# tsinghua-fib-lab/DRL-urban-planning

Measured on NVIDIA H100. Metric: ppo_update_graph_samples_per_sec, higher is better.
Workload: dtype f32

## Files before the change

drl_urban_planning_b200/csrc/mlp_kernel.cuh:

```cuda
#pragma once
#include "sgnn_kernel.cuh"

namespace upb {

constexpr int M_NUM_W0 = 0;
constexpr int M_NUM_B0 = 3328;
constexpr int M_NUM_W1 = 3392;
constexpr int M_NUM_B1 = 4416;
constexpr int M_ENC_W = 4432;
constexpr int M_ENC_B = 4800;
constexpr int M_LU_W0 = 4816;
constexpr int M_LU_B0 = 6864;
constexpr int M_LU_W1 = 6896;
constexpr int M_RD_W0 = 6928;
constexpr int M_RD_B0 = 7440;
constexpr int M_RD_W1 = 7472;
constexpr int M_SVD = 51;
constexpr int M_VAL_W0 = 7504;
constexpr int M_VAL_B0 = 9136;
constexpr int M_VAL_W1 = 9168;
constexpr int M_VAL_B1 = 10192;
constexpr int M_VAL_W2 = 10224;
constexpr int M_VAL_B2 = 10256;
constexpr int M_NUM_PARAMS = 10257;
// ... 364 lines not shown
    float s0 = 0.f, s1 = 0.f;
    int i = 0;
    for (; i + 1 < n; i += 2) {
      s0 = fmaf(GH[(size_t)i * 16 + c], X[(size_t)i * FS + f], s0);
      s1 = fmaf(GH[(size_t)(i + 1) * 16 + c], X[(size_t)(i + 1) * FS + f], s1);
    }
    if (i < n) s0 = fmaf(GH[(size_t)i * 16 + c], X[(size_t)i * FS + f], s0);
    gacc(gp, M_ENC_W + idx, (s0 + s1) + sV[MV_GHC + c] * sV[MV_XCUR + f]);
  }
  if (tid < 16) gacc(gp, M_ENC_B + tid, sV[MV_T16 + tid] + sV[MV_GHC + tid]);
  __syncthreads();
}

constexpr int M_NSLICE = MlpRow::nslice;
static_assert(M_NSLICE == 81 && MG_ROW - (M_NSLICE - 1) * SLICE == 64,
              "tests/test_gpu_mlp_step.py runs the rl-mlp fused tail at grids of 80 / 81 / 82 CTAs around M_NSLICE: move them");
static_assert(M_NSLICE * SLICE <= G_ROW && M_NSLICE <= FLAG_STRIDE, "the SGNN exchange buffer holds the rl-mlp row");
static_assert(MT == 2 * SLICE, "two threads per column of a slice");

__device__ void mlp_fused_tail(const StepArgs& a, float* smem, unsigned stage_bits) {
  const int tid = threadIdx.x;
  const int nparts = gridDim.x;
  const int world = a.world, me = a.rank;
  const bool sys = world > 1;
  const unsigned par = a.seq & 1u;
  __shared__ TailShared sh;
  float* const mine = a.peers[me];
  const float* const pull = mine + (size_t)par * MAX_PEERS * G_ROW;
  const unsigned* const myflags = reinterpret_cast<const unsigned*>(mine + XCHG_FLAGS) + (size_t)par * MAX_PEERS * FLAG_STRIDE;
  tail_prologue(a, sh, stage_bits);
  const int c = tid & (SLICE - 1), half = tid >> 7;
  const int col0 = blockIdx.x * SLICE + c;
  float pm = 0.f, pv = 0.f, pp = 0.f;
  if (half == 0 && col0 < M_NUM_PARAMS) { pm = a.adam_m[col0]; pv = a.adam_v[col0]; pp = a.params_rw[col0]; }
  const unsigned flagword = tail_barrier(a);

  float* sHalf = smem;
  const int nq = nparts & ~3;
  for (int sl = blockIdx.x; sl < M_NSLICE; sl += gridDim.x) {
    const int col = sl * SLICE + c;
    const bool in_row = col < MG_ROW;
    const float* src = a.gpart + col + (size_t)(2 * half) * MG_ROW;
    float sa = 0.f, sb = 0.f;
    if (in_row) {
      int r = 0;
      for (; r + 16 <= nq; r += 16) {
        float t[8];
#pragma unroll
        for (int j = 0; j < 4; ++j) {
          t[2 * j] = __ldcg(src + (size_t)(r + 4 * j) * MG_ROW);
          t[2 * j + 1] = __ldcg(src + (size_t)(r + 4 * j + 1) * MG_ROW);
        }
#pragma unroll
        for (int j = 0; j < 4; ++j) { sa += t[2 * j]; sb += t[2 * j + 1]; }
      }
      for (; r < nq; r += 4) {
        const float x0 = __ldcg(src + (size_t)r * MG_ROW), x1 = __ldcg(src + (size_t)(r + 1) * MG_ROW);
        sa += x0; sb += x1;
      }
      if (half == 0)
        for (r = nq; r < nparts; ++r) sa += __ldcg(src + (size_t)r * MG_ROW);
    }
    const float pair = sa + sb;
    __syncthreads();
    if (half) sHalf[c] = pair;
    __syncthreads();
    if (half == 0 && in_row) {
      const float v = pair + sHalf[c];
      for (int r = 0; r < world; ++r) st_relaxed(sh.push[r] + col, v, sys);
    }
  }
  tail_release<MlpRow>(a, flagword, MT, sys);
  if (a.kl_stop) tail_kl_gate<MlpRow>(a, sh, pull, myflags, sys);

  tail_reduce_adam<MlpRow>(a, sh, pull, myflags, sys, c, half == 0, col0, pm, pv, pp);
  if (blockIdx.x == 0 && tid < 4) tail_write_steps(a, sh);
  tail_count_timeout(a, sh);
}

template <bool TRAIN>
__global__ void __launch_bounds__(MT, 1) k_mlp(const __grid_constant__ StepArgs a) {
  extern __shared__ __align__(16) float smem[];
  __shared__ __align__(8) uint64_t s_mbar[1];
  if constexpr (TRAIN) {
    if (a.kl_stop && kl_stop_set(a.kl_stop)) {
      skip_step<MlpRow>(a);
      return;
    }
  }
  if (threadIdx.x == 0) { mbar_init(s_mbar, 1); fence_mbar_init(); }
  for (int i = threadIdx.x; i < 10272; i += MT) smem[MS_P + i] = i < M_NUM_PARAMS ? a.params[i] : 0.f;
  for (int i = threadIdx.x; i < 384; i += MT) {
    const int f = i >> 4, c = i & 15;
    smem[MS_WET + i] = f < F ? a.params[M_ENC_W + c * F + f] : 0.f;
  }
  float* gp = nullptr;
  if constexpr (TRAIN) {
    gp = a.gpart + (size_t)blockIdx.x * MG_ROW;
    for (int i = threadIdx.x; i < MG_ROW; i += MT) gp[i] = 0.f;
  }
  __syncthreads();
  const BlobHeader& hd = *reinterpret_cast<const BlobHeader*>(a.blob);
  const GraphDesc* descs = reinterpret_cast<const GraphDesc*>(a.blob + hd.off_desc);
  float* scr = a.scratch + (size_t)blockIdx.x * a.scratch_stride;
  unsigned nstaged = 0;
  unsigned stage_bits = 0;
  for (int item = blockIdx.x; item < a.count; item += gridDim.x) {
    const int gid = a.ids ? a.ids[item] : item;
    const GraphDesc d = descs[gid];
    if (d.n > a.n_cap || d.e > a.e_cap || d.n < 1) {
      if (threadIdx.x == 0) {
        if constexpr (TRAIN) gp[MG_STATS + 7] += 1.f;
        if (a.out_value) a.out_value[gid] = CUDART_NAN_F;
        if (a.out_logp) a.out_logp[gid] = CUDART_NAN_F;
        if (a.out_entropy) a.out_entropy[gid] = CUDART_NAN_F;
      }
      if constexpr (!TRAIN) write_skipped_logit_row<MT>(a, gid, d.stage);
      continue;
    }
    stage_bits |= d.stage == 0 ? 1u : (d.stage == 1 ? 2u : 0u);
    const bool big = d.n > M_NS || 2 * d.e > M_AS || d.k > M_KS;
    mlp_graph<TRAIN>(a, hd, d, gid, smem, gp, scr, s_mbar, nstaged & 1u, big);
    if (!big) ++nstaged;
    __syncthreads();
  }
  if constexpr (TRAIN) {
    if (a.fuse_tail) mlp_fused_tail(a, smem, stage_bits);
  }
}

__global__ void __launch_bounds__(256) k_mlp_reduce(const float* __restrict__ gpart, int nparts, float* __restrict__ grad,
                                                    const unsigned int* kl_stop) {
  const int idx = blockIdx.x * 256 + threadIdx.x;
  if (kl_stop && kl_stop_set(kl_stop)) {
    if (idx < UPB_MLP_GRAD_STRIDE) write_skip_elem(grad, UPB_MLP_STAT_OFFSET, idx);
    return;
  }
  if (idx >= MG_ROW) return;
  write_grad_col<MlpRow>(grad, idx, column_sum4<MlpRow>(gpart, nparts, idx));
}

}
```

drl_urban_planning_b200/csrc/sgnn_kernel.cuh:

```cuda
#pragma once
#include <cuda_runtime.h>
#include <math_constants.h>
#include <stdint.h>

#include "blob.h"
#include "layout.h"
#include "optim_kernels.cuh"

namespace upb {

constexpr int NT = 512;
constexpr int NW = NT / 32;
constexpr int NS = 464;
constexpr int AS = 5632;
constexpr int KS = 160;
constexpr int CH = 96;
constexpr float MASK_FILL = -4294967296.0f;
constexpr float EPS_DEG = 1e-6f;

constexpr int S_WET = 0;
constexpr int S_BE = S_WET + 384;
constexpr int S_WPQ0 = S_BE + 16;
constexpr int S_B0 = S_WPQ0 + 512;
constexpr int S_WPQ1 = S_B0 + 16;
// ... 128 lines not shown
  const float* fixed_lp;
  const float* exps;
  float inv_batch, inv_ind;
  float clip_lo, clip_hi;
  float c_value, c_entropy;
  int diagnostics;
  float* out_value;
  float* out_logp;
  float* out_entropy;
  int* out_greedy;
  const float* uniforms;
  int* out_sample;
  float* gpart;
  float* scratch;
  size_t scratch_stride;
  int n_cap, e_cap;
  int fuse_tail;
  float* params_rw;
  float* grad_out;
  float* adam_m;
  float* adam_v;
  const long long* steps_in;
  long long* steps_out;
  unsigned int* gridbar;
  unsigned int bar_target;
  float lr, beta1, beta2, adam_eps;
  float weight_decay;
  int world, rank;
  unsigned int seq;
  float* const* peers;
  long long* stamps;
  const int* logit_rows;
  float* lu_logits;
  float* rd_logits;
  unsigned int* kl_stop;
  float kl_limit;
};

__device__ __forceinline__ float ex2_approx(float x) {
  float y;
  asm("ex2.approx.ftz.f32 %0, %1;" : "=f"(y) : "f"(x));
  return y;
}
__device__ __forceinline__ float rcp_approx(float x) {
  float y;
  asm("rcp.approx.ftz.f32 %0, %1;" : "=f"(y) : "f"(x));
  return y;
}
__device__ __forceinline__ float exp2a(float a) {
  const float t = fminf(fmaxf(a * 2.8853900817779268f, -115.41560327111707f), 115.41560327111707f);
  return ex2_approx(t);
}
__device__ __forceinline__ void cp_async16(void* smem_dst, const void* gsrc) {
  const unsigned d = (unsigned)__cvta_generic_to_shared(smem_dst);
  asm volatile("cp.async.cg.shared.global [%0], [%1], 16;" ::"r"(d), "l"(gsrc) : "memory");
}
__device__ __forceinline__ void cp_async_commit() { asm volatile("cp.async.commit_group;" ::: "memory"); }
__device__ __forceinline__ void cp_async_wait_all() { asm volatile("cp.async.wait_group 0;" ::: "memory"); }

__device__ __forceinline__ unsigned smem_u32(const void* p) { return (unsigned)__cvta_generic_to_shared(p); }
__device__ __forceinline__ void mbar_init(uint64_t* bar, unsigned count) {
  asm volatile("mbarrier.init.shared::cta.b64 [%0], %1;" ::"r"(smem_u32(bar)), "r"(count) : "memory");
}
__device__ __forceinline__ void fence_mbar_init() { asm volatile("fence.mbarrier_init.release.cluster;" ::: "memory"); }
__device__ __forceinline__ void fence_proxy_async() { asm volatile("fence.proxy.async;" ::: "memory"); }
__device__ __forceinline__ void mbar_expect_tx(uint64_t* bar, unsigned bytes) {
  asm volatile("mbarrier.arrive.expect_tx.shared::cta.b64 _, [%0], %1;" ::"r"(smem_u32(bar)), "r"(bytes) : "memory");
}
__device__ __forceinline__ void bulk_g2s(void* smem_dst, const void* gsrc, unsigned bytes, uint64_t* bar) {
  asm volatile("cp.async.bulk.shared::cluster.global.mbarrier::complete_tx::bytes [%0], [%1], %2, [%3];"
               ::"r"(smem_u32(smem_dst)), "l"(gsrc), "r"(bytes), "r"(smem_u32(bar)) : "memory");
}
__device__ __forceinline__ void mbar_wait(uint64_t* bar, unsigned parity) {
  asm volatile(
      "{\n\t.reg .pred p;\n\t"
      "WAIT_%=:\n\t"
      "mbarrier.try_wait.parity.shared::cta.b64 p, [%0], %1;\n\t"
      "@p bra DONE_%=;\n\t"
      "bra WAIT_%=;\n\t"
      "DONE_%=:\n\t}"
      ::"r"(smem_u32(bar)), "r"(parity) : "memory");
}

__device__ __forceinline__ float4 ld4(const float* p) { return *reinterpret_cast<const float4*>(p); }
__device__ __forceinline__ void st4(float* p, float4 v) { *reinterpret_cast<float4*>(p) = v; }
__device__ __forceinline__ float4 f4(float a) { return make_float4(a, a, a, a); }
__device__ __forceinline__ float4 operator+(float4 a, float4 b) { return make_float4(a.x + b.x, a.y + b.y, a.z + b.z, a.w + b.w); }
__device__ __forceinline__ float4 operator*(float4 a, float s) { return make_float4(a.x * s, a.y * s, a.z * s, a.w * s); }
__device__ __forceinline__ float4 operator*(float4 a, float4 b) { return make_float4(a.x * b.x, a.y * b.y, a.z * b.z, a.w * b.w); }
__device__ __forceinline__ float dot4(float4 a, float4 b) { return a.x * b.x + a.y * b.y + a.z * b.z + a.w * b.w; }
__device__ __forceinline__ float comp(const float4& v, int j) { return j == 0 ? v.x : j == 1 ? v.y : j == 2 ? v.z : v.w; }

struct F2x2 { float2 a, b; };
__device__ __forceinline__ float2 ffma2(float2 a, float2 b, float2 c) {
  return make_float2(__fmaf_rn(a.x, b.x, c.x), __fmaf_rn(a.y, b.y, c.y));
}
__device__ __forceinline__ float2 fmul2(float2 a, float2 b) { return make_float2(__fmul_rn(a.x, b.x), __fmul_rn(a.y, b.y)); }
__device__ __forceinline__ float2 fadd2(float2 a, float2 b) { return make_float2(__fadd_rn(a.x, b.x), __fadd_rn(a.y, b.y)); }
__device__ __forceinline__ F2x2 ldp(const float* p) {
  const float4 v = ld4(p);
  F2x2 r; r.a = make_float2(v.x, v.y); r.b = make_float2(v.z, v.w);
  return r;
}
template <bool SM>
struct RowBase {
  const float* p;
  unsigned a;
  __device__ __forceinline__ explicit RowBase(const float* base) : p(base), a(SM ? smem_u32(base) : 0u) {}
  __device__ __forceinline__ F2x2 row(unsigned k, int shift) const {
    if constexpr (SM) {
      float4 v;
      asm volatile("ld.shared.v4.f32 {%0, %1, %2, %3}, [%4];" : "=f"(v.x), "=f"(v.y), "=f"(v.z), "=f"(v.w) : "r"(a + (k << shift)));
      F2x2 r; r.a = make_float2(v.x, v.y); r.b = make_float2(v.z, v.w);
      return r;
    } else {
      return ldp(reinterpret_cast<const float*>(reinterpret_cast<const char*>(p) + ((size_t)k << shift)));
    }
  }
};
__device__ __forceinline__ float2 rcp2(float2 v) { return make_float2(rcp_approx(v.x), rcp_approx(v.y)); }
__device__ __forceinline__ float2 neg2(float2 v) { return make_float2(-v.x, -v.y); }

template <int TIER>
__device__ __forceinline__ float2 edge_den(float2 p, float2 q) {
  if constexpr (TIER == 2) {
    const float2 x = fadd2(p, q);
    return make_float2(__fadd_rn(exp2a(x.x), 1.f), __fadd_rn(exp2a(x.y), 1.f));
  } else {
    return ffma2(p, q, make_float2(1.f, 1.f));
  }
}
template <int TIER>
__device__ __forceinline__ void fwd_term(float2 epi, float2 eqi, float2 epk, float2 eqk, float2& s) {
  const float2 a = edge_den<TIER>(epi, eqk), b = edge_den<TIER>(epk, eqi);
  if (TIER > 0) s = fadd2(s, fadd2(rcp2(a), rcp2(b)));
  else s = ffma2(fadd2(a, b), rcp2(fmul2(a, b)), s);
}
template <int TIER>
__device__ __forceinline__ void bwd_term(float2 epi, float2 eqi, float2 epk, float2 eqk, float2 ge2, float2& aP,
                                         float2& aQ) {
  const float2 one = make_float2(1.f, 1.f);
  const float2 a = edge_den<TIER>(epi, eqk), b = edge_den<TIER>(epk, eqi);
  float2 r1, r2;
  if (TIER > 0) { r1 = rcp2(a); r2 = rcp2(b); }
  else { const float2 R = rcp2(fmul2(a, b)); r1 = fmul2(b, R); r2 = fmul2(a, R); }
  aP = ffma2(ge2, fmul2(r1, fadd2(one, neg2(r1))), aP);
  aQ = ffma2(ge2, fmul2(r2, fadd2(one, neg2(r2))), aQ);
}

__device__ __forceinline__ float warp_sum(float v) {
#pragma unroll
  for (int o = 16; o > 0; o >>= 1) v += __shfl_xor_sync(0xffffffffu, v, o);
  return v;
}
__device__ __forceinline__ float warp_max(float v) {
#pragma unroll
  for (int o = 16; o > 0; o >>= 1) v = fmaxf(v, __shfl_xor_sync(0xffffffffu, v, o));
  return v;
}

__device__ __forceinline__ float block_sum1(float v, float* red) {
  v = warp_sum(v);
  if ((threadIdx.x & 31) == 0) red[threadIdx.x >> 5] = v;
  __syncthreads();
  float s = 0.f;
#pragma unroll
// ... 1499 lines not shown
constexpr unsigned PEER_SPIN_LIMIT = 1u << 24;

__device__ __forceinline__ float ld_relaxed(const float* p, bool sys) {
  float v;
  if (sys) asm volatile("ld.relaxed.sys.global.f32 %0, [%1];" : "=f"(v) : "l"(p));
  else asm volatile("ld.relaxed.gpu.global.f32 %0, [%1];" : "=f"(v) : "l"(p));
  return v;
}
__device__ __forceinline__ void st_relaxed(float* p, float v, bool sys) {
  if (sys) asm volatile("st.relaxed.sys.global.f32 [%0], %1;" ::"l"(p), "f"(v) : "memory");
  else asm volatile("st.relaxed.gpu.global.f32 [%0], %1;" ::"l"(p), "f"(v) : "memory");
}
__device__ __forceinline__ unsigned ld_acquire(const unsigned* p, bool sys) {
  unsigned v;
  if (sys) asm volatile("ld.acquire.sys.global.u32 %0, [%1];" : "=r"(v) : "l"(p) : "memory");
  else asm volatile("ld.acquire.gpu.global.u32 %0, [%1];" : "=r"(v) : "l"(p) : "memory");
  return v;
}
__device__ __forceinline__ void st_release(unsigned* p, unsigned v, bool sys) {
  if (sys) asm volatile("st.release.sys.global.u32 [%0], %1;" ::"l"(p), "r"(v) : "memory");
  else asm volatile("st.release.gpu.global.u32 [%0], %1;" ::"l"(p), "r"(v) : "memory");
}

__device__ __forceinline__ void grid_arrive(unsigned int* ctr) {
  __syncthreads();
  if (threadIdx.x == 0) {
    __threadfence();
    atomicAdd(ctr, 1u);
  }
}
__device__ __forceinline__ void grid_wait(unsigned int* ctr, unsigned int target) {
  if (threadIdx.x == 0) {
    unsigned int v;
    do {
      asm volatile("ld.acquire.gpu.global.u32 %0, [%1];" : "=r"(v) : "l"(ctr) : "memory");
    } while ((int)(v - target) < 0);
    __threadfence();
  }
  __syncthreads();
}

__device__ __forceinline__ void adam_elem(const StepArgs& a, int i, float g, float m, float v, float p, float step_size,
                                          float bc2_sqrt) {
  const float w1 = 1.f - a.beta1, w2 = 1.f - a.beta2;
  if (a.weight_decay != 0.f) g = __fmaf_rn(a.weight_decay, p, g);
  m = __fadd_rn(m, __fmul_rn(w1, __fsub_rn(g, m)));
  v = __fadd_rn(__fmul_rn(v, a.beta2), __fmul_rn(__fmul_rn(w2, g), g));
  const float denom = __fadd_rn(__fdiv_rn(__fsqrt_rn(v), bc2_sqrt), a.adam_eps);
  a.params_rw[i] = __fadd_rn(p, __fmul_rn(-step_size, __fdiv_rn(m, denom)));
  a.adam_m[i] = m;
  a.adam_v[i] = v;
}

struct TailShared {
  float adam[12];
  long long steps[6];
  unsigned bits;
  int timeout;
  int stop;
  float* push[MAX_PEERS];
};

__device__ __forceinline__ void tail_prologue(const StepArgs& a, TailShared& sh, unsigned stage_bits) {
  const int tid = threadIdx.x;
  const unsigned par = a.seq & 1u;
  if (tid < a.world) sh.push[tid] = a.peers[tid] + ((size_t)par * MAX_PEERS + a.rank) * G_ROW;
  if (tid == 32) { sh.timeout = 0; sh.bits = 0u; sh.stop = 0; }
  if (tid == 0 && stage_bits) atomicOr(a.gridbar + 2 + par, stage_bits);
  if (tid == 1 && blockIdx.x == 0) a.gridbar[2 + (par ^ 1u)] = 0u;
  if (tid < 6) {
    const int seg = tid >> 1, live = tid & 1;
    const long long stp = a.steps_in[1 + seg] + live;
    const double bc1 = 1.0 - ipow((double)a.beta1, stp > 0 ? stp : 1);
    const double bc2 = 1.0 - ipow((double)a.beta2, stp > 0 ? stp : 1);
    sh.adam[tid * 2 + 0] = (float)((double)a.lr / bc1);
    sh.adam[tid * 2 + 1] = (float)sqrt(bc2);
    sh.steps[tid] = stp;
  }
}

__device__ __forceinline__ unsigned tail_barrier(const StepArgs& a) {
  grid_arrive(a.gridbar);
  grid_wait(a.gridbar, a.bar_target);
  unsigned mybits;
  asm volatile("ld.acquire.gpu.global.u32 %0, [%1];" : "=r"(mybits) : "l"(a.gridbar + 2 + (a.seq & 1u)) : "memory");
  return (a.seq << 2) | (mybits & 3u);
}

template <class L>
__device__ __forceinline__ void tail_release(const StepArgs& a, unsigned flagword, int nthreads, bool sys) {
  __syncthreads();
  const unsigned par = a.seq & 1u;
  const int nown = (L::nslice - (int)blockIdx.x + (int)gridDim.x - 1) / (int)gridDim.x;
  for (int idx = threadIdx.x; idx < a.world * nown; idx += nthreads) {
    const int r = idx % a.world, sl = blockIdx.x + (idx / a.world) * gridDim.x;
    unsigned* f = reinterpret_cast<unsigned*>(a.peers[r] + XCHG_FLAGS) + ((size_t)par * MAX_PEERS + a.rank) * FLAG_STRIDE + sl;
    if (sys) __threadfence_system(); else __threadfence();
    st_release(f, flagword, sys);
  }
}

__device__ __forceinline__ void tail_poll(const StepArgs& a, TailShared& sh, const unsigned* myflags, int r, int sl,
                                          bool sys) {
  unsigned polls = 0, f;
  while ((int)(((f = ld_acquire(myflags + (size_t)r * FLAG_STRIDE + sl, sys)) >> 2) - a.seq) < 0) {
    if (++polls >= PEER_SPIN_LIMIT) { sh.timeout = 1; break; }
  }
  if (f & 3u) atomicOr(&sh.bits, f & 3u);
}

template <class L>
__device__ __forceinline__ void tail_reduce_adam(const StepArgs& a, TailShared& sh, const float* pull,
                                                 const unsigned* myflags, bool sys, int c, bool active, int col0,
                                                 float pm, float pv, float pp) {
  const int world = a.world;
  for (int sl = blockIdx.x; sl < L::nslice; sl += gridDim.x) {
    if ((int)threadIdx.x < world) tail_poll(a, sh, myflags, threadIdx.x, sl, sys);
    __syncthreads();
    const bool live_lu = sh.bits & 1u, live_rd = sh.bits & 2u;
    const bool dead = sh.timeout != 0 || sh.stop;
    const int col = sl * SLICE + c;
    if (active && (L::row % SLICE == 0 || col < L::row)) {
      float v[MAX_PEERS];
#pragma unroll
      for (int p = 0; p < MAX_PEERS; ++p) v[p] = p < world ? ld_relaxed(pull + (size_t)p * G_ROW + col, sys) : 0.f;
      float s = v[0];
#pragma unroll
      for (int p = 1; p < MAX_PEERS; ++p) if (p < world) s += v[p];
      if (write_grad_col<L>(a.grad_out, col, s)) {
        int seg = 0;
        bool live = true;
        if (col >= L::lu_begin && col < L::rd_begin) { seg = 1; live = live_lu; }
        else if (col >= L::rd_begin && col < L::policy_end) { seg = 2; live = live_rd; }
        if (live && !dead) {
          if (col != col0) { pm = a.adam_m[col]; pv = a.adam_v[col]; pp = a.params_rw[col]; }
          adam_elem(a, col, s, pm, pv, pp, sh.adam[(seg * 2 + 1) * 2], sh.adam[(seg * 2 + 1) * 2 + 1]);
        }
      } else if (sh.stop && col == L::stats + KL_STOP_SLOT) {
        a.grad_out[L::stat_offset + KL_STOP_SLOT] = 1.f;
        *a.kl_stop = 1u;
      }
    }
    __syncthreads();
  }
}

__device__ __forceinline__ void tail_write_steps(const StepArgs& a, const TailShared& sh) {
  const int tid = threadIdx.x;
  const bool live_lu = sh.bits & 1u, live_rd = sh.bits & 2u;
  if (sh.timeout == 0 && !sh.stop)
    a.steps_out[tid] = tid == 0 ? a.steps_in[0] + 1
                                : sh.steps[(tid - 1) * 2 + (tid == 1 ? 1 : (tid == 2 ? (live_lu ? 1 : 0) : (live_rd ? 1 : 0)))];
  else
    a.steps_out[tid] = a.steps_in[tid];
}

__device__ __forceinline__ void tail_count_timeout(const StepArgs& a, const TailShared& sh) {
  if (threadIdx.x == 0 && sh.timeout) atomicAdd(a.gridbar + 6, 1u);
}

template <class L>
__device__ __noinline__ void tail_kl_gate(const StepArgs& a, TailShared& sh, const float* pull, const unsigned* myflags,
                                          bool sys) {
  if ((int)threadIdx.x < a.world) tail_poll(a, sh, myflags, threadIdx.x, L::stats / SLICE, sys);
  __syncthreads();
  if (threadIdx.x == 0) {
// ... 66 lines not shown
    }
  }
  const unsigned flagword = tail_barrier(a);
  UPB_TSTAMP(41);

  float* sPart = smem + 4096;
  for (int sl = blockIdx.x; sl < NSLICE; sl += gridDim.x) {
    const int lane = tid & 31, warp = tid >> 5, cg = warp & 3, rg = warp >> 2;
    const float* src = a.gpart + sl * SLICE + cg * 32 + lane;
    float s = 0.f;
    for (int r0 = rg; r0 < nparts; r0 += 160) {
      float t[40];
#pragma unroll
      for (int j = 0; j < 40; ++j) t[j] = r0 + 4 * j < nparts ? __ldcg(src + (size_t)(r0 + 4 * j) * G_ROW) : 0.f;
#pragma unroll
      for (int w = 1; w < 40; w <<= 1)
#pragma unroll
        for (int j = 0; j + w < 40; j += 2 * w) t[j] += t[j + w];
      s += t[0];
    }
    __syncthreads();
    sPart[rg * SLICE + cg * 32 + lane] = s;
    __syncthreads();
    if (tid < SLICE) {
      const float v = (sPart[tid] + sPart[SLICE + tid]) + (sPart[2 * SLICE + tid] + sPart[3 * SLICE + tid]);
      const int col = sl * SLICE + tid;
      for (int r = 0; r < world; ++r) st_relaxed(sh.push[r] + col, v, sys);
    }
  }
  tail_release<SgnnRow>(a, flagword, NT, sys);
  if (a.kl_stop) tail_kl_gate<SgnnRow>(a, sh, pull, myflags, sys);
  UPB_TSTAMP(42);

  tail_reduce_adam<SgnnRow>(a, sh, pull, myflags, sys, tid >> 2, part == 0, col0, pm, pv, pp);
  UPB_TSTAMP(43);
  if (!chain_cta) {
    tail_count_timeout(a, sh);
    return;
  }

  {
    constexpr int NCH = CHAIN_S1 - CHAIN_S0 + 1;
    if (tid < world * NCH) tail_poll(a, sh, myflags, tid % world, CHAIN_S0 + tid / world, sys);
    __syncthreads();
  }
  const bool dead = sh.timeout != 0 || sh.stop;
  if (tid < 4) tail_write_steps(a, sh);
  {
    float v0[MAX_PEERS], v1[MAX_PEERS];
#pragma unroll
    for (int p = 0; p < MAX_PEERS; ++p) {
      v0[p] = 0.f; v1[p] = 0.f;
      if (p < world) {
        v0[p] = ld_relaxed(pull + (size_t)p * G_ROW + G_QC + tid, sys);
        if (tid + NT < 816) v1[p] = ld_relaxed(pull + (size_t)p * G_ROW + G_QC + tid + NT, sys);
      }
    }
    float s0 = v0[0], s1 = v1[0];
#pragma unroll
    for (int p = 1; p < MAX_PEERS; ++p) if (p < world) { s0 += v0[p]; s1 += v1[p]; }
    sG[tid] = s0;
    if (tid + NT < 816) sG[tid + NT] = s1;
  }
  __syncthreads();
  if (tid < 256) attention_chain(tid, sG, sWin, sW3, sB, sOut, 256, sOut + 768, sOut + 1536, 16, sOut + 1584);
  __syncthreads();
#pragma unroll
  for (int j = 0; j < 4; ++j) {
    const int i = tid + j * NT;
    if (i < 1632) {
      const float g = sOut[i];
      a.grad_out[cdst[j]] = g;
      if (!dead) adam_elem(a, cdst[j], g, cm[j], cv[j], cp[j], sh.adam[2], sh.adam[3]);
    }
  }
  tail_count_timeout(a, sh);
  UPB_TSTAMP(44);
}

template <bool TRAIN>
__global__ void __launch_bounds__(NT, 1) k_sgnn(const __grid_constant__ StepArgs a) {
  extern __shared__ __align__(16) float smem[];
  __shared__ __align__(8) uint64_t s_mbar[4];
  if constexpr (TRAIN) {
    if (a.kl_stop && kl_stop_set(a.kl_stop)) {
      skip_step<SgnnRow>(a);
      return;
    }
  }
  const long long t_cta0 = a.stamps ? clock64() : 0;
  if (a.stamps && threadIdx.x == 0 && blockIdx.x == 0) {
    unsigned long long gt;
    asm volatile("mov.u64 %0, %%globaltimer;" : "=l"(gt));
    a.stamps[30] = t_cta0; a.stamps[32] = (long long)gt;
  }
  if (threadIdx.x == 0) {
    mbar_init(s_mbar + 0, 1); mbar_init(s_mbar + 1, 1); mbar_init(s_mbar + 2, 1); mbar_init(s_mbar + 3, 1);
    fence_mbar_init();
  }
  unsigned nstaged = 0;
  load_weights(a.params, smem);
  float* gp = nullptr;
  if constexpr (TRAIN) {
    gp = a.gpart + (size_t)blockIdx.x * G_ROW;
    for (int i = threadIdx.x; i < G_ROW / 4; i += NT) reinterpret_cast<float4*>(gp)[i] = f4(0.f);
  }
  __syncthreads();
  if (a.stamps && threadIdx.x == 0 && blockIdx.x < 160) a.stamps[64 + 160 + blockIdx.x] = clock64() - t_cta0;
  const BlobHeader& hd = *reinterpret_cast<const BlobHeader*>(a.blob);
  const GraphDesc* descs = reinterpret_cast<const GraphDesc*>(a.blob + hd.off_desc);
  float* scr = a.scratch + (size_t)blockIdx.x * a.scratch_stride;
  unsigned stage_bits = 0;
  for (int item = blockIdx.x; item < a.count; item += gridDim.x) {
    const int gid = a.ids ? a.ids[item] : item;
    const GraphDesc d = descs[gid];
    stage_bits |= 1u << (d.stage & 1);
    if (d.n > a.n_cap || d.e > a.e_cap || d.n < 1) {
      if (threadIdx.x == 0) {
        if constexpr (TRAIN) gacc(gp, G_STATS + 7, 1.f);
        if (a.out_value) a.out_value[gid] = CUDART_NAN_F;
        if (a.out_logp) a.out_logp[gid] = CUDART_NAN_F;
        if (a.out_entropy) a.out_entropy[gid] = CUDART_NAN_F;
      }
      if constexpr (!TRAIN) write_skipped_logit_row<NT>(a, gid, d.stage);
      continue;
    }
    if (item + (int)gridDim.x < a.count) prefetch_next_graph<TRAIN>(a, item + gridDim.x);
    const bool big = d.n > NS || 2 * d.e > AS || d.k > KS || d.ord_rounds > ORD_ROUNDS;
    if (big) graph_body<TRAIN, true>(a, hd, d, gid, smem, gp, scr, item == (int)(blockIdx.x + gridDim.x), s_mbar, 0u);
    else { graph_body<TRAIN, false>(a, hd, d, gid, smem, gp, scr, item == (int)(blockIdx.x + gridDim.x), s_mbar, nstaged & 1u); ++nstaged; }
    __syncthreads();
  }
  if (a.stamps && threadIdx.x == 0 && blockIdx.x < 160) a.stamps[64 + blockIdx.x] = clock64() - t_cta0;
  if (a.stamps && threadIdx.x == 0 && blockIdx.x == 0) {
    unsigned long long gt;
    asm volatile("mov.u64 %0, %%globaltimer;" : "=l"(gt));
    a.stamps[31] = clock64(); a.stamps[33] = (long long)gt;
  }
  if constexpr (TRAIN) {
    if (a.fuse_tail) fused_tail(a, smem, stage_bits);
  }
}

}
```

drl_urban_planning_b200/csrc/upb200.cu:

```cuda
#include <cuda_runtime.h>

#include <cmath>
#include <cstdio>
#include <cstring>
#include <new>
#include <string>
#include <utility>
#include <vector>

#include "../../include/upb200.h"
#include "blob.h"
#include "errors.h"
#include "layout.h"
#include "optim_kernels.cuh"
#include "sgnn_kernel.cuh"
#include "mlp_kernel.cuh"

using namespace upb;

struct Model {
  void (*train)(StepArgs);
  void (*infer)(StepArgs);
  int threads;
  size_t smem;
  int row;
  int num_params, encoder_end, policy_end, lu_begin, rd_begin, stat_offset, grad_stride;
  size_t (*scratch_floats)(int n_cap, int e_cap);
  void (*reduce)(const upb_ctx* ctx, int nparts, const float* params, float* grad, const unsigned int* kl_stop,
                 cudaStream_t s);
  bool peer_exchange;

  float* gpart = nullptr;
  float* scratch = nullptr;
  size_t scratch_stride = 0;
  float* adam_m = nullptr;
  float* adam_v = nullptr;
  long long* steps = nullptr;
  unsigned int* kl_stop = nullptr;
  int steps_cur = 0;
  bool clip_armed = true;
};

namespace {
void reduce_sgnn(const upb_ctx* ctx, int nparts, const float* params, float* grad, const unsigned int* kl_stop,
                 cudaStream_t s);
void reduce_mlp(const upb_ctx* ctx, int nparts, const float* params, float* grad, const unsigned int* kl_stop,
                cudaStream_t s);
}

struct upb_ctx {
  upb_config cfg;
  int num_sms = 0;
  int grid = 0;
  Model sgnn{k_sgnn<true>, k_sgnn<false>, NT, SMEM_BYTES, G_ROW, NUM_PARAMS, ENCODER_END, POLICY_END, P_LU_W0,
             P_RD_W0, UPB_STAT_OFFSET, UPB_GRAD_STRIDE, scratch_floats, reduce_sgnn, true};
  Model mlp{k_mlp<true>, k_mlp<false>, MT, M_SMEM_BYTES, MG_ROW, M_NUM_PARAMS, M_ENCODER_END, M_POLICY_END, M_LU_W0,
            M_RD_W0, UPB_MLP_STAT_OFFSET, UPB_MLP_GRAD_STRIDE, mlp_scratch_floats, reduce_mlp, false};
  float* gsum = nullptr;
  unsigned int* ticket = nullptr;
  unsigned int* gridbar = nullptr;
  unsigned int bar_total = 0;
  float weight_decay = 0.f;
  bool diagnostics = false;
  float kl_limit = 0.f;
  float clip_lo = 0.f, clip_hi = 0.f;
  int coop = 0;
  float* host_pinned = nullptr;
  int64_t launches = 0;
  bool profiling = false;
  long long* stamps = nullptr;
  std::vector<std::pair<cudaEvent_t, cudaEvent_t>> prof_events;
  size_t prof_used = 0;
  float* xchg = nullptr;
  int world = 1, rank = 0;
  unsigned int peer_seq = 0;
  std::vector<void*> peer_ptrs;
  float** peers_dev = nullptr;
};

namespace {

#define UPB_CUDA(call)                                                                       \
  do {                                                                                       \
    cudaError_t err__ = (call);                                                              \
    if (err__ != cudaSuccess) {                                                              \
      char buf__[512];                                                                       \
      snprintf(buf__, sizeof(buf__), "%s failed: %s (%s:%d)", #call, cudaGetErrorString(err__), \
               __FILE__, __LINE__);                                                          \
      return set_error(UPB_ERR_CUDA, buf__);                                                 \
    }                                                                                        \
  } while (0)

struct Slot {
  const char* name;
  int offset, rows, cols;
};
const Slot kSlots[] = {
    {"num_w0", P_NUM_W0, 64, 52},      {"num_b0", P_NUM_B0, 64, 0},     {"num_w1", P_NUM_W1, 16, 64},
    {"num_b1", P_NUM_B1, 16, 0},       {"enc_w", P_ENC_W, 16, 23},      {"enc_b", P_ENC_B, 16, 0},
    {"gcn0_w", P_GCN0_W, 16, 32},      {"gcn0_b", P_GCN0_B, 16, 0},     {"gcn1_w", P_GCN1_W, 16, 32},
    {"gcn1_b", P_GCN1_B, 16, 0},       {"mha_in_w", P_MHA_IN_W, 48, 16}, {"mha_in_b", P_MHA_IN_B, 48, 0},
    {"mha_out_w", P_MHA_OUT_W, 16, 16}, {"mha_out_b", P_MHA_OUT_B, 16, 0}, {"att_q_w", P_ATT_Q_W, 16, 16},
    {"att_q_b", P_ATT_Q_B, 16, 0},     {"att_k_w", P_ATT_K_W, 16, 16},  {"att_k_b", P_ATT_K_B, 16, 0},
    {"att_v_w", P_ATT_V_W, 16, 16},    {"att_v_b", P_ATT_V_B, 16, 0},   {"lu_w0", P_LU_W0, 32, 64},
    {"lu_b0", P_LU_B0, 32, 0},         {"lu_w1", P_LU_W1, 1, 32},       {"road_w0", P_RD_W0, 32, 16},
    {"road_b0", P_RD_B0, 32, 0},       {"road_w1", P_RD_W1, 1, 32},     {"val_w0", P_VAL_W0, 32, 67},
    {"val_b0", P_VAL_B0, 32, 0},       {"val_w1", P_VAL_W1, 32, 32},    {"val_b1", P_VAL_B1, 32, 0},
    {"val_w2", P_VAL_W2, 1, 32},       {"val_b2", P_VAL_B2, 1, 0},
};
constexpr int kNumSlots = sizeof(kSlots) / sizeof(kSlots[0]);

using ModelOf = Model upb_ctx::*;

int check_ctx(const upb_ctx* ctx, const char* who) {
  if (!ctx) return set_error(UPB_ERR_ARG, std::string(who) + ": null context");
  return UPB_OK;
}
int bad_argument(const char* who) { return set_error(UPB_ERR_ARG, std::string(who) + ": bad argument"); }

bool prof_begin(upb_ctx* ctx, cudaStream_t s) {
  if (!ctx->profiling) return false;
  if (ctx->prof_used == ctx->prof_events.size()) {
    cudaEvent_t a, b;
    if (cudaEventCreate(&a) != cudaSuccess || cudaEventCreate(&b) != cudaSuccess) return false;
    ctx->prof_events.emplace_back(a, b);
  }
  cudaEventRecord(ctx->prof_events[ctx->prof_used].first, s);
  return true;
}
void prof_end(upb_ctx* ctx, cudaStream_t s, bool on) {
  if (!on) return;
  cudaEventRecord(ctx->prof_events[ctx->prof_used].second, s);
  ctx->prof_used += 1;
}

bool clip_now(const upb_ctx* ctx, const Model& m) {
  return ctx->cfg.clip_mode == UPB_CLIP_ALWAYS || (ctx->cfg.clip_mode == UPB_CLIP_REFERENCE && m.clip_armed);
}

int model_init(upb_ctx* ctx, Model& m) {
  if (m.gpart) return UPB_OK;
  m.scratch_stride = (m.scratch_floats(ctx->cfg.n_cap, ctx->cfg.e_cap) + 63) & ~size_t(63);
  UPB_CUDA(cudaMalloc(&m.gpart, sizeof(float) * (size_t)ctx->grid * m.row));
  UPB_CUDA(cudaMalloc(&m.scratch, sizeof(float) * (size_t)ctx->grid * m.scratch_stride));
  UPB_CUDA(cudaMalloc(&m.adam_m, sizeof(float) * m.num_params));
  UPB_CUDA(cudaMalloc(&m.adam_v, sizeof(float) * m.num_params));
  UPB_CUDA(cudaMalloc(&m.steps, sizeof(long long) * 8));
  UPB_CUDA(cudaMalloc(&m.kl_stop, sizeof(unsigned int)));
  UPB_CUDA(cudaMemset(m.kl_stop, 0, sizeof(unsigned int)));
  UPB_CUDA(cudaMemset(m.adam_m, 0, sizeof(float) * m.num_params));
  UPB_CUDA(cudaMemset(m.adam_v, 0, sizeof(float) * m.num_params));
  UPB_CUDA(cudaMemset(m.steps, 0, sizeof(long long) * 8));
  UPB_CUDA(cudaMemset(m.scratch, 0, sizeof(float) * (size_t)ctx->grid * m.scratch_stride));
  UPB_CUDA(cudaFuncSetAttribute(m.train, cudaFuncAttributeMaxDynamicSharedMemorySize, (int)m.smem));
  UPB_CUDA(cudaFuncSetAttribute(m.infer, cudaFuncAttributeMaxDynamicSharedMemorySize, (int)m.smem));
  UPB_CUDA(cudaDeviceSynchronize());
  return UPB_OK;
}

void model_free(Model& m) {
  cudaFree(m.gpart);
  cudaFree(m.scratch);
  cudaFree(m.adam_m);
  cudaFree(m.adam_v);
  cudaFree(m.steps);
  cudaFree(m.kl_stop);
}

void reduce_sgnn(const upb_ctx* ctx, int nparts, const float* params, float* grad, const unsigned int* kl_stop,
                 cudaStream_t s) {
  k_reduce_finish<<<RF_BLOCKS, RF_THREADS, 0, s>>>(ctx->sgnn.gpart, nparts, ctx->gsum, params, grad, ctx->ticket,
                                                   kl_stop);
}
void reduce_mlp(const upb_ctx* ctx, int nparts, const float*, float* grad, const unsigned int* kl_stop,
                cudaStream_t s) {
  k_mlp_reduce<<<(MG_ROW + 255) / 256, 256, 0, s>>>(ctx->mlp.gpart, nparts, grad, kl_stop);
}

unsigned int* kl_stop_word(const upb_ctx* ctx, const Model& m) { return ctx->kl_limit > 0.f ? m.kl_stop : nullptr; }

StepArgs step_args(const upb_ctx* ctx, const Model& m, const void* blob, const int32_t* ids, int count,
                   const float* params, const float* actions) {
  StepArgs a;
  memset(&a, 0, sizeof(a));
  a.blob = (const uint8_t*)blob;
  a.ids = ids;
  a.count = count;
  a.params = params;
  a.actions = actions;
  a.clip_lo = ctx->clip_lo;
  a.clip_hi = ctx->clip_hi;
  a.c_value = ctx->cfg.value_pred_coef;
  a.c_entropy = ctx->cfg.entropy_coef;
  a.diagnostics = ctx->diagnostics ? 1 : 0;
  a.gpart = m.gpart;
  a.scratch = m.scratch;
  a.scratch_stride = m.scratch_stride;
  a.n_cap = ctx->cfg.n_cap;
  a.e_cap = ctx->cfg.e_cap;
  a.stamps = ctx->stamps;
  return a;
}

void set_ppo_inputs(StepArgs& a, const float* advantages, const float* returns, const float* fixed_log_probs,
                    const float* exps, float inv_batch, float inv_ind) {
  a.adv = advantages;
  a.ret = returns;
  a.fixed_lp = fixed_log_probs;
  a.exps = exps;
  a.inv_batch = inv_batch;
  a.inv_ind = inv_ind;
}

void set_kl_stop(StepArgs& a, const upb_ctx* ctx, const Model& m) {
  a.kl_stop = kl_stop_word(ctx, m);
  a.kl_limit = ctx->kl_limit;
}

int forward(upb_ctx* ctx, ModelOf model, const char* who, const void* blob_dev, const int32_t* ids, int count,
            const float* params, const float* actions, float* value, float* log_prob, float* entropy, int32_t* greedy,
            const int32_t* logit_rows, float* lu_logits, float* rd_logits, cudaStream_t s) {
  if (int rc = check_ctx(ctx, who)) return rc;
  if (!blob_dev || !params || count < 0) return bad_argument(who);
  Model& m = ctx->*model;
  if (int rc = model_init(ctx, m)) return rc;
  if (count == 0) return UPB_OK;
  StepArgs a = step_args(ctx, m, blob_dev, ids, count, params, actions);
  a.out_value = value;
  a.out_logp = log_prob;
  a.out_entropy = entropy;
  a.out_greedy = greedy;
  a.logit_rows = logit_rows;
  a.lu_logits = lu_logits;
  a.rd_logits = rd_logits;
  const int grid = count < ctx->grid ? count : ctx->grid;
  const bool prof = prof_begin(ctx, s);
  m.infer<<<grid, m.threads, m.smem, s>>>(a);
  prof_end(ctx, s, prof);
  ctx->launches += 1;
  UPB_CUDA(cudaGetLastError());
// ... 48 lines not shown
  m.reduce(ctx, grid, params, grad_out, a.kl_stop, s);
  ctx->launches += 1;
  UPB_CUDA(cudaGetLastError());
  return UPB_OK;
}

int apply(upb_ctx* ctx, ModelOf model, const char* who, float* params, float* grad, cudaStream_t s) {
  if (int rc = check_ctx(ctx, who)) return rc;
  if (!params || !grad) return bad_argument(who);
  Model& m = ctx->*model;
  if (int rc = model_init(ctx, m)) return rc;
  ApplyArgs a;
  a.params = params;
  a.grad = grad;
  a.m = m.adam_m;
  a.v = m.adam_v;
  a.steps_in = m.steps + 4 * m.steps_cur;
  a.steps_out = m.steps + 4 * (1 - m.steps_cur);
  m.steps_cur = 1 - m.steps_cur;
  a.lr = ctx->cfg.lr;
  a.beta1 = ctx->cfg.beta1;
  a.beta2 = ctx->cfg.beta2;
  a.eps = ctx->cfg.adam_eps;
  a.weight_decay = ctx->weight_decay;
  a.clip_now = clip_now(ctx, m) ? 1 : 0;
  m.clip_armed = false;
  a.num_params = m.num_params; a.encoder_end = m.encoder_end; a.policy_end = m.policy_end;
  a.lu_begin = m.lu_begin; a.rd_begin = m.rd_begin; a.stat_offset = m.stat_offset;
  a.kl_stop = kl_stop_word(ctx, m);
  a.kl_limit = ctx->kl_limit;
  k_apply<<<AP_BLOCKS, AP_THREADS, 0, s>>>(a);
  ctx->launches += 1;
  UPB_CUDA(cudaGetLastError());
  return UPB_OK;
}

int ppo_step(upb_ctx* ctx, ModelOf model, const char* who, const char* grad_who, const char* apply_who,
             const void* blob_dev, const int32_t* ids, int count, float* params, const float* actions,
             const float* advantages, const float* returns, const float* fixed_log_probs, const float* exps,
             float inv_batch, float inv_ind, float* grad_out, cudaStream_t s) {
  if (int rc = check_ctx(ctx, who)) return rc;
  Model& m = ctx->*model;
  const bool clip_step = clip_now(ctx, m);
  if (ctx->world > 1) {
    if (!m.peer_exchange)
      return set_error(UPB_ERR_ARG, std::string(who) + ": peers are connected; rl-mlp multi-GPU steps use "
                                                       "upb_mlp_ppo_grad + all-reduce + upb_mlp_apply");
    if (clip_step || !ctx->coop)
      return set_error(UPB_ERR_ARG, std::string(who) + ": peers are connected and this step clips gradients; use "
                                                       "upb_ppo_grad + all-reduce + upb_apply for it "
                                                       "(upb_next_step_fused() == 0)");
  } else if (clip_step || !ctx->coop || count <= 0) {
    int rc = ppo_grad(ctx, model, grad_who, blob_dev, ids, count, params, actions, advantages, returns,
                      fixed_log_probs, exps, inv_batch, inv_ind, grad_out, s);
    if (rc != UPB_OK) return rc;
    return apply(ctx, model, apply_who, params, grad_out, s);
  }
  if (!blob_dev || !params || !actions || !advantages || !returns || !fixed_log_probs || !exps || !grad_out)
    return bad_argument(who);
  if (int rc = model_init(ctx, m)) return rc;
  StepArgs a = step_args(ctx, m, blob_dev, ids, count, params, actions);
  set_ppo_inputs(a, advantages, returns, fixed_log_probs, exps, inv_batch, inv_ind);
  set_kl_stop(a, ctx, m);
  a.fuse_tail = 1;
  a.params_rw = params;
  a.grad_out = grad_out;
  a.adam_m = m.adam_m;
  a.adam_v = m.adam_v;
  a.steps_in = m.steps + 4 * m.steps_cur;
  a.steps_out = m.steps + 4 * (1 - m.steps_cur);
  a.gridbar = ctx->gridbar;
  a.lr = ctx->cfg.lr;
  a.beta1 = ctx->cfg.beta1;
  a.beta2 = ctx->cfg.beta2;
  a.adam_eps = ctx->cfg.adam_eps;
  a.weight_decay = ctx->weight_decay;
  a.world = ctx->world;
  a.rank = ctx->rank;
  a.seq = ++ctx->peer_seq;
  a.peers = ctx->peers_dev;
  const int grid = count < 1 ? 1 : (count < ctx->grid ? count : ctx->grid);
  ctx->bar_total += (unsigned int)grid;
  a.bar_target = ctx->bar_total;
  void* kargs[] = {&a};
  const bool prof = prof_begin(ctx, s);
  UPB_CUDA(cudaLaunchCooperativeKernel((void*)m.train, dim3(grid), dim3(m.threads), kargs, m.smem, s));
  prof_end(ctx, s, prof);
  ctx->launches += 1;
  m.steps_cur = 1 - m.steps_cur;
  m.clip_armed = false;
  return UPB_OK;
}

int next_step_fused(upb_ctx* ctx, ModelOf model) {
  if (!ctx) return 0;
  const Model& m = ctx->*model;
  return ((m.peer_exchange || ctx->world == 1) && !clip_now(ctx, m) && ctx->coop) ? 1 : 0;
}

int rearm_clip(upb_ctx* ctx, ModelOf model, const char* who) {
  if (int rc = check_ctx(ctx, who)) return rc;
  (ctx->*model).clip_armed = true;
  return UPB_OK;
}

int reset_kl_stop(upb_ctx* ctx, ModelOf model, const char* who, cudaStream_t s) {
  if (int rc = check_ctx(ctx, who)) return rc;
  Model& m = ctx->*model;
  if (int rc = model_init(ctx, m)) return rc;
  UPB_CUDA(cudaMemsetAsync(m.kl_stop, 0, sizeof(unsigned int), s));
  return UPB_OK;
}

int read_losses(upb_ctx* ctx, ModelOf model, const char* who, const float* grad, float* out4_host, cudaStream_t s) {
  if (int rc = check_ctx(ctx, who)) return rc;
  if (!grad || !out4_host) return bad_argument(who);
  UPB_CUDA(cudaMemcpyAsync(ctx->host_pinned, grad + (ctx->*model).stat_offset, sizeof(float) * 8,
                           cudaMemcpyDeviceToHost, s));
  UPB_CUDA(cudaStreamSynchronize(s));
  const float* st = ctx->host_pinned;
  const float nB = st[3] > 0.f ? st[3] : 1.f, nI = st[4] > 0.f ? st[4] : 1.f;
  const float value_loss = st[0] / nB, surr = st[1] / nI, ent = st[2] / nI;
  out4_host[0] = surr + ctx->cfg.value_pred_coef * value_loss + ctx->cfg.entropy_coef * ent;
  out4_host[1] = value_loss;
  out4_host[2] = surr;
  out4_host[3] = ent;
  return UPB_OK;
}

int get_opt_state(upb_ctx* ctx, ModelOf model, const char* who, float* m_host, float* v_host, int64_t* steps4_host) {
  if (int rc = check_ctx(ctx, who)) return rc;
  Model& m = ctx->*model;
  if (int rc = model_init(ctx, m)) return rc;
  UPB_CUDA(cudaDeviceSynchronize());
  if (m_host) UPB_CUDA(cudaMemcpy(m_host, m.adam_m, sizeof(float) * m.num_params, cudaMemcpyDeviceToHost));
  if (v_host) UPB_CUDA(cudaMemcpy(v_host, m.adam_v, sizeof(float) * m.num_params, cudaMemcpyDeviceToHost));
  if (steps4_host)
    UPB_CUDA(cudaMemcpy(steps4_host, m.steps + 4 * m.steps_cur, sizeof(long long) * 4, cudaMemcpyDeviceToHost));
  return UPB_OK;
}

int set_opt_state(upb_ctx* ctx, ModelOf model, const char* who, const float* m_host, const float* v_host,
                  const int64_t* steps4_host) {
  if (int rc = check_ctx(ctx, who)) return rc;
  Model& m = ctx->*model;
  if (int rc = model_init(ctx, m)) return rc;
  UPB_CUDA(cudaDeviceSynchronize());
  if (m_host) UPB_CUDA(cudaMemcpy(m.adam_m, m_host, sizeof(float) * m.num_params, cudaMemcpyHostToDevice));
  if (v_host) UPB_CUDA(cudaMemcpy(m.adam_v, v_host, sizeof(float) * m.num_params, cudaMemcpyHostToDevice));
  if (steps4_host) {
    UPB_CUDA(cudaMemcpy(m.steps + 4 * m.steps_cur, steps4_host, sizeof(long long) * 4, cudaMemcpyHostToDevice));
    m.clip_armed = steps4_host[0] == 0;
  }
  return UPB_OK;
}

int grad_norms(upb_ctx* ctx, ModelOf model, const char* who, const float* grad_rows, int rows, float* out,
               cudaStream_t s) {
  if (int rc = check_ctx(ctx, who)) return rc;
  if (!grad_rows || !out || rows < 0) return bad_argument(who);
  if (rows == 0) return UPB_OK;
  const Model& m = ctx->*model;
  k_grad_norms<<<rows, GN_THREADS, 0, s>>>(grad_rows, m.grad_stride, m.num_params, m.encoder_end, m.policy_end, out);
  ctx->launches += 1;
  UPB_CUDA(cudaGetLastError());
  return UPB_OK;
}

}
// ... 321 lines not shown
```

Before: 1.780 million.

## Launch fused step kernels with programmatic dependent launch and early graph prefetch

```diff
diff --git a/drl_urban_planning_b200/csrc/mlp_kernel.cuh b/drl_urban_planning_b200/csrc/mlp_kernel.cuh
--- a/drl_urban_planning_b200/csrc/mlp_kernel.cuh
+++ b/drl_urban_planning_b200/csrc/mlp_kernel.cuh
@@ -470,6 +470,7 @@
 __global__ void __launch_bounds__(MT, 1) k_mlp(const __grid_constant__ StepArgs a) {
   extern __shared__ __align__(16) float smem[];
   __shared__ __align__(8) uint64_t s_mbar[1];
+  grid_dep_wait();
   if constexpr (TRAIN) {
     if (a.kl_stop && kl_stop_set(a.kl_stop)) {
       skip_step<MlpRow>(a);
diff --git a/drl_urban_planning_b200/csrc/sgnn_kernel.cuh b/drl_urban_planning_b200/csrc/sgnn_kernel.cuh
--- a/drl_urban_planning_b200/csrc/sgnn_kernel.cuh
+++ b/drl_urban_planning_b200/csrc/sgnn_kernel.cuh
@@ -234,6 +234,9 @@
       ::"r"(smem_u32(bar)), "r"(parity) : "memory");
 }
 
+__device__ __forceinline__ void grid_dep_wait() { asm volatile("griddepcontrol.wait;" ::: "memory"); }
+__device__ __forceinline__ void grid_dep_launch() { asm volatile("griddepcontrol.launch_dependents;" ::: "memory"); }
+
 __device__ __forceinline__ float4 ld4(const float* p) { return *reinterpret_cast<const float4*>(p); }
 __device__ __forceinline__ void st4(float* p, float4 v) { *reinterpret_cast<float4*>(p) = v; }
 __device__ __forceinline__ float4 f4(float a) { return make_float4(a, a, a, a); }
@@ -1899,6 +1902,7 @@
 __device__ __forceinline__ unsigned tail_barrier(const StepArgs& a) {
   grid_arrive(a.gridbar);
   grid_wait(a.gridbar, a.bar_target);
+  grid_dep_launch();
   unsigned mybits;
   asm volatile("ld.acquire.gpu.global.u32 %0, [%1];" : "=r"(mybits) : "l"(a.gridbar + 2 + (a.seq & 1u)) : "memory");
   return (a.seq << 2) | (mybits & 3u);
@@ -2131,6 +2135,8 @@
 __global__ void __launch_bounds__(NT, 1) k_sgnn(const __grid_constant__ StepArgs a) {
   extern __shared__ __align__(16) float smem[];
   __shared__ __align__(8) uint64_t s_mbar[4];
+  if ((int)blockIdx.x < a.count) prefetch_next_graph<TRAIN>(a, blockIdx.x);
+  grid_dep_wait();
   if constexpr (TRAIN) {
     if (a.kl_stop && kl_stop_set(a.kl_stop)) {
       skip_step<SgnnRow>(a);
diff --git a/drl_urban_planning_b200/csrc/upb200.cu b/drl_urban_planning_b200/csrc/upb200.cu
--- a/drl_urban_planning_b200/csrc/upb200.cu
+++ b/drl_urban_planning_b200/csrc/upb200.cu
@@ -39,6 +39,7 @@
   unsigned int* kl_stop = nullptr;
   int steps_cur = 0;
   bool clip_armed = true;
+  bool step_pdl = false;
 };
 
 namespace {
@@ -154,8 +155,33 @@
   UPB_CUDA(cudaMemset(m.scratch, 0, sizeof(float) * (size_t)ctx->grid * m.scratch_stride));
   UPB_CUDA(cudaFuncSetAttribute(m.train, cudaFuncAttributeMaxDynamicSharedMemorySize, (int)m.smem));
   UPB_CUDA(cudaFuncSetAttribute(m.infer, cudaFuncAttributeMaxDynamicSharedMemorySize, (int)m.smem));
+  int per_sm = 0;
+  UPB_CUDA(cudaOccupancyMaxActiveBlocksPerMultiprocessor(&per_sm, m.train, m.threads, m.smem));
+  m.step_pdl = per_sm * ctx->num_sms >= ctx->grid;
   UPB_CUDA(cudaDeviceSynchronize());
   return UPB_OK;
+}
+
+cudaError_t launch_step(Model& m, int grid, StepArgs& a, cudaStream_t s) {
+  void* kargs[] = {&a};
+  cudaLaunchAttribute attr;
+  cudaLaunchConfig_t lc = {};
+  lc.gridDim = dim3(grid);
+  lc.blockDim = dim3(m.threads);
+  lc.dynamicSmemBytes = m.smem;
+  lc.stream = s;
+  lc.attrs = &attr;
+  lc.numAttrs = 1;
+  if (m.step_pdl) {
+    attr.id = cudaLaunchAttributeProgrammaticStreamSerialization;
+    attr.val.programmaticStreamSerializationAllowed = 1;
+    if (cudaLaunchKernelExC(&lc, (const void*)m.train, kargs) == cudaSuccess) return cudaSuccess;
+    cudaGetLastError();
+    m.step_pdl = false;
+  }
+  attr.id = cudaLaunchAttributeCooperative;
+  attr.val.cooperative = 1;
+  return cudaLaunchKernelExC(&lc, (const void*)m.train, kargs);
 }
 
 void model_free(Model& m) {
@@ -370,9 +396,8 @@
   const int grid = count < 1 ? 1 : (count < ctx->grid ? count : ctx->grid);
   ctx->bar_total += (unsigned int)grid;
   a.bar_target = ctx->bar_total;
-  void* kargs[] = {&a};
   const bool prof = prof_begin(ctx, s);
-  UPB_CUDA(cudaLaunchCooperativeKernel((void*)m.train, dim3(grid), dim3(m.threads), kargs, m.smem, s));
+  UPB_CUDA(launch_step(m, grid, a, s));
   prof_end(ctx, s, prof);
   ctx->launches += 1;
   m.steps_cur = 1 - m.steps_cur;
```

After: 1.818 million, median of 6. +2.1%, better.
